# CarbonMatrixLab/AbX

Measured on AMD Instinct MI355X. Metric: diffusion-steps/sec (100 samples, ~350-res complex), higher is better.
Workload: dtype f32; 1 GPU; L352: L=352 (Lab 228 + antigen 124), 100 samples of one complex over 1 GPU(s), 1 step = ScoreNetwork (3 passes) + get_prev + reverse, seeded random weights, ESM off; L=352, samples_total=100, chunk=auto, parallelism=sample-shard x1, no collective in the step

## Files before the change

abx_amd/_lib.py:

```python
import ctypes as C
import os

_HERE = os.path.dirname(os.path.abspath(__file__))
LIB_PATH = os.environ.get('ABX_HIP_LIB') or os.path.join(_HERE, 'csrc', 'libabx_hip.so')

c_f = C.c_void_p
LL = C.c_longlong
I = C.c_int
F = C.c_float


class AbxGemm(C.Structure):
    _fields_ = [
        ('A', c_f), ('sAb', LL), ('sAm', LL), ('sAk', LL),
        ('B', c_f), ('sBb', LL), ('sBk', LL), ('sBn', LL),
        ('C', c_f), ('sCb', LL), ('sCm', LL),
        ('M', I), ('N', I), ('K', I), ('batch', I),
        ('c_transposed', I),
        ('ln_stats', c_f), ('sSb', LL),
        ('ln_csum', c_f),
        ('ln_eps', F),
        ('a_relu', I),
        ('bias', c_f),
        ('alpha', F),
# ... 300 lines not shown
        ('out', c_f), ('out_stride', LL),
        ('bonds', c_f), ('rows', c_f),
        ('B', I), ('L', I), ('Lab', I),
    ]


_S = c_f

_PROTOS = {
    'abx_version': (I, []),
    'abx_last_error_string': (C.c_char_p, []),
    'abx_init': (I, [I]),
    'abx_gemm': (I, [C.POINTER(AbxGemm), _S]),
    'abx_gemm_side': (I, [C.POINTER(AbxGemm), C.POINTER(AbxGemm), _S]),
    'abx_gemm_check_modes': (I, [C.POINTER(AbxGemm)]),
    'abx_gemm_planes_ok': (I, [LL]),
    'abx_split_weights_f16': (I, [c_f, LL, LL, I, I, I, C.c_void_p, _S]),
    'abx_ipa_tail': (I, [C.POINTER(AbxIpaTail), _S]),
    'abx_heads_tail': (I, [C.POINTER(AbxHeadsTail), _S]),
    'abx_gemm3_occupancy': (I, [I]),
    'abx_row_stats': (I, [c_f, LL, LL, LL, I, I, I, F, c_f, _S]),
    'abx_layernorm': (I, [c_f, LL, LL, I, c_f, c_f, F, c_f, LL, c_f, LL, _S]),
    'abx_tri_attn_fwd': (I, [C.POINTER(AbxTriAttn), _S]),
    'abx_tri_rowpack_bytes': (LL, []),
    'abx_tri_rowpack': (I, [C.POINTER(AbxLinearPack), c_f, C.POINTER(AbxTriRowPack), _S]),
    'abx_tri_attn_rowfused_ok': (I, [I]),
    'abx_tri_attn_rowfused_fwd': (I, [C.POINTER(AbxTriAttn), c_f, LL, LL, LL, C.POINTER(AbxTriRowPack), I, _S]),
    'abx_seq_attn_fwd': (I, [c_f, c_f, c_f, c_f, c_f, I, I, I, I, F, _S]),
    'abx_ipa_pack': (I, [c_f, c_f, c_f, c_f, c_f, c_f, I, I, F, _S]),
    'abx_ipa_attn': (I, [c_f, c_f, c_f, c_f, c_f, c_f, c_f, c_f, c_f, c_f, c_f, I, I, _S]),
    'abx_debug_poison_lds': (I, [C.c_uint, _S]),
    'abx_ipa_weights': (I, [c_f, c_f, c_f, c_f, c_f, c_f, c_f, c_f, c_f, c_f, I, I, _S]),
    'abx_ipa_pair': (I, [c_f, c_f, c_f, I, I, _S]),
    'abx_ipa_attn_workspace_bytes': (C.c_longlong, [I, I]),
    'abx_ipa_qpack_bytes': (C.c_longlong, [I, I]),
    'abx_timestep_embedding': (I, [c_f, c_f, I, I, c_f, _S]),
    'abx_assemble_seq': (I, [c_f, LL, c_f, c_f, I, c_f, c_f, c_f, c_f, c_f, I, I, I, I, _S]),
    'abx_assemble_pair': (I, [c_f, LL, c_f, c_f, c_f, c_f, c_f, c_f, c_f, c_f, I, I, I, I, _S]),
    'abx_opm_features': (I, [c_f, c_f, LL, c_f, I, I, I, _S]),
    'abx_opm_out_fwd': (I, [c_f, LL, c_f, c_f, c_f, I, I, c_f, I, _S]),
    'abx_assemble_pair_bias': (I, [c_f, LL, c_f, c_f, c_f, c_f, c_f, c_f, c_f, C.c_void_p, I, c_f, c_f, F, c_f, I, I, c_f, I, _S]),
    'abx_pair_mask': (I, [c_f, c_f, I, I, I, _S]),
    'abx_transpose_last2': (I, [c_f, c_f, I, I, I, I, _S]),
    'abx_pair_embed_features': (I, [c_f, c_f, c_f, c_f, c_f, c_f, c_f, c_f, c_f, c_f, c_f, c_f, I, I, _S]),
    'abx_relpos_block': (I, [c_f, c_f, c_f, I, I, I, I, I, _S]),
    'abx_gather_rows': (I, [c_f, c_f, c_f, c_f, LL, LL, I, _S]),
    'abx_frames_init': (I, [c_f, I, c_f, c_f, c_f, c_f, c_f, c_f, I, F, _S]),
    'abx_rigid_update': (I, [c_f, c_f, c_f, c_f, c_f, c_f, c_f, c_f, I, F, _S]),
    'abx_scores': (I, [C.POINTER(AbxScoreArgs), _S]),
    'abx_torsion_finalize': (I, [c_f, c_f, c_f, c_f, I, _S]),
    'abx_seq_head_atoms': (I, [c_f, c_f, c_f, c_f, c_f, c_f, c_f, c_f, c_f, c_f, c_f, c_f, I, _S]),
    'abx_prev_pos': (I, [c_f, c_f, I, c_f, I, I, _S]),
    'abx_plddt': (I, [c_f, c_f, I, I, _S]),
    'abx_igso3_tables': (I, [c_f, c_f, I, I, I, c_f, c_f, c_f, _S]),
    'abx_reverse_step': (I, [C.POINTER(AbxReverseArgs), _S]),
    'abx_clash_grad_workspace_bytes': (LL, [I, I]),
    'abx_clash_grad': (I, [C.POINTER(AbxGuidanceArgs), c_f, _S]),
    'abx_contact_grad_workspace_bytes': (LL, [I, I, I]),
    'abx_contact_grad': (I, [C.POINTER(AbxContactArgs), c_f, _S]),
    'abx_design_scores_workspace_bytes': (LL, [I, I]),
    'abx_design_scores': (I, [C.POINTER(AbxDesignScoreArgs), c_f, _S]),
    'abx_relax_workspace_bytes': (LL, [I, I, I]),
    'abx_relax_lds_bytes': (LL, [I, I]),
    'abx_relax': (I, [C.POINTER(AbxRelaxArgs), c_f, _S]),
    'abx_interface_scores_workspace_bytes': (LL, [I, I, I]),
    'abx_interface_scores': (I, [C.POINTER(AbxInterfaceArgs), c_f, _S]),
# ... 55 lines not shown
```

abx_amd/csrc/ipa.hip:

```cpp
#include "common.h"
#include "abx_hip.h"

namespace {

constexpr int H = 12, SQK = 16, SV = 16, PQK = 4, PV = 8, CZ = 128;
constexpr int QREC = SQK + 3 * PQK;
constexpr int VREC = SV + 3 * PV;
constexpr int NPROJ = H * SQK + H * (SQK + SV) + 3 * H * PQK + 3 * H * (PQK + PV);
constexpr int OFF_KV = H * SQK;
constexpr int OFF_QP = OFF_KV + H * (SQK + SV);
constexpr int OFF_KVP = OFF_QP + 3 * H * PQK;
constexpr int NFEAT = H * SV + 3 * H * PV + H * PV + H * CZ;

constexpr int IPA_THREADS = 512;
constexpr int IQ = 12;
constexpr int HG = 4, NHG = H / HG;

__global__ __launch_bounds__(256) void ipa_pack_kernel(const float* __restrict__ proj, const float* __restrict__ rots,
                                                       const float* __restrict__ trans, float* __restrict__ qpack,
                                                       float* __restrict__ kpack, float* __restrict__ vpack, int B, int L,
                                                       float w_s) {
    const int NIB = (L + IQ - 1) / IQ, LQ = NIB * IQ;
    const long long idx = (long long)blockIdx.x * 256 + threadIdx.x;
    if (idx >= (long long)B * LQ * H) return;
// ... 26 lines not shown
        float x[3];
#pragma unroll
        for (int r = 0; r < 3; ++r) x[r] = p[OFF_QP + r * (H * PQK) + h * PQK + pt];
#pragma unroll
        for (int r = 0; r < 3; ++r) q[2 * (SQK + pt * 3 + r)] = t[r] + (R[r * 3 + 0] * x[0] + R[r * 3 + 1] * x[1] + R[r * 3 + 2] * x[2]);
    }
#pragma unroll
    for (int pt = 0; pt < PQK + PV; ++pt) {
        float x[3], y[3];
#pragma unroll
        for (int r = 0; r < 3; ++r) x[r] = p[OFF_KVP + r * (H * (PQK + PV)) + h * (PQK + PV) + pt];
#pragma unroll
        for (int r = 0; r < 3; ++r) y[r] = t[r] + (R[r * 3 + 0] * x[0] + R[r * 3 + 1] * x[1] + R[r * 3 + 2] * x[2]);
        if (pt < PQK) {
#pragma unroll
            for (int r = 0; r < 3; ++r) k[SQK + pt * 3 + r] = y[r];
        } else {
#pragma unroll
            for (int r = 0; r < 3; ++r) v[SV + (pt - PQK) * 3 + r] = y[r];
        }
    }
}

__host__ __device__ inline int ipa_row_stride(int L) { return ((L + 31) / 32) * 32 + 12; }
constexpr int RED_I = IQ * 4 + 4;
constexpr int RED_G = (HG * VREC / 4) * RED_I + 4;
__host__ __device__ inline size_t ipa_logits_floats(int L) {
    const size_t lgf = (size_t)IQ * HG * ipa_row_stride(L), redf = (size_t)6 * RED_G;
    return lgf > redf ? lgf : redf;
}

#ifdef IPA_STAMP
__device__ unsigned long long ipa_stamp_buf[1024 * 8];
#define ISTAMP(k) { if (threadIdx.x == 0 && blockIdx.x >= 4096 && blockIdx.x < 5120) ipa_stamp_buf[(blockIdx.x - 4096) * 8 + (k)] = __builtin_amdgcn_s_memtime(); }
#else
#define ISTAMP(k) {}
#endif
__global__ __launch_bounds__(IPA_THREADS, 4) void ipa_weights_kernel(const float* __restrict__ qpack, const float* __restrict__ kpack,
                                                                     const float* __restrict__ vpack, const float* __restrict__ bias2d,
                                                                     const float* __restrict__ mask, const float* __restrict__ rots,
                                                                     const float* __restrict__ trans, const float* __restrict__ pw,
                                                                     float* __restrict__ attn, float* __restrict__ feat, int B, int L) {
    extern __shared__ __attribute__((aligned(16))) float smem[];
    const int LR = ipa_row_stride(L);
    float* lg = smem;
    float* opt = smem + ipa_logits_floats(L);
    const int tid = threadIdx.x, lane = tid & 63, wave = tid >> 6;
    const int NIB = (L + IQ - 1) / IQ, per_b = NIB * NHG;
    const int xcd = blockIdx.x & 7, slot = blockIdx.x >> 3;
    const int full_slots = (B / 8) * per_b;
    int b, wb;
    if (slot < full_slots) {
        b = (slot / per_b) * 8 + xcd;
        wb = slot % per_b;
    } else {
        const int t = (slot - full_slots) * 8 + xcd;
        if (t >= (B % 8) * per_b) return;
        b = (B / 8) * 8 + t / per_b;
        wb = t % per_b;
    }
    const int hg = wb % NHG, h0 = hg * HG;
    const int iblk = wb / NHG;
    const int i0 = iblk * IQ;
    const int niq = min(IQ, L - i0);

    ISTAMP(0)
    {
        typedef float f32x2 __attribute__((ext_vector_type(2)));
        const float* __restrict__ qb = qpack + (((long long)b * NIB + iblk) * H + h0) * (IQ / 2) * (QREC * 2);
        const int wpk = (L + 63) >> 6;
        for (int task = wave; task < HG * wpk; task += IPA_THREADS / 64) {
            const int hl = __builtin_amdgcn_readfirstlane(task / wpk);
            const int j = (task - hl * wpk) * 64 + lane;
            const float* kr = kpack + (((long long)b * H + h0 + hl) * L + min(j, L - 1)) * QREC;
            f32x4 kq[QREC / 4];
#pragma unroll
            for (int c4 = 0; c4 < QREC / 4; ++c4) kq[c4] = *reinterpret_cast<const f32x4*>(kr + c4 * 4);
            const float pwh = pw[h0 + hl];
            const f32x2* __restrict__ qh = reinterpret_cast<const f32x2*>(qb + (long long)hl * (IQ / 2) * (QREC * 2));
#pragma unroll
            for (int ip = 0; ip < IQ / 2; ++ip) {
                f32x2 sacc = {0.f, 0.f}, d2 = {0.f, 0.f};
// ... 144 lines not shown
        }
        if (jg == 0) {
#pragma unroll
            for (int iq = 0; iq < IQ; ++iq) *reinterpret_cast<f32x4*>(opt + (size_t)(iq * HG + hl1) * VREC + c41 * 4) = acc[iq];
        }
        __syncthreads();
    }
    ISTAMP(6)
    for (int idx = tid; idx < niq * HG * SV; idx += IPA_THREADS) {
        const int iq = idx / (HG * SV), r = idx % (HG * SV);
        feat[((long long)b * L + i0 + iq) * NFEAT + h0 * SV + r] = opt[(iq * HG + r / SV) * VREC + (r % SV)];
    }
    for (int idx = tid; idx < niq * HG * PV; idx += IPA_THREADS) {
        const int iq = idx / (HG * PV), nl = idx % (HG * PV);
        const int hl = nl / PV, pt = nl % PV, n = h0 * PV + nl;
        const long long row = (long long)b * L + i0 + iq;
        const float* R = rots + row * 9;
        const float* t = trans + row * 3;
        const float* g = opt + (iq * HG + hl) * VREC + SV + pt * 3;
        float loc[3];
#pragma unroll
        for (int r = 0; r < 3; ++r) {
            const float it = -(R[0 * 3 + r] * t[0] + R[1 * 3 + r] * t[1] + R[2 * 3 + r] * t[2]);
            loc[r] = it + (R[0 * 3 + r] * g[0] + R[1 * 3 + r] * g[1] + R[2 * 3 + r] * g[2]);
        }
        float* fo = feat + row * NFEAT;
#pragma unroll
        for (int r = 0; r < 3; ++r) fo[H * SV + r * (H * PV) + n] = loc[r];
        fo[H * SV + 3 * H * PV + n] = sqrtf(loc[0] * loc[0] + loc[1] * loc[1] + loc[2] * loc[2] + 1e-8f);
    }
    ISTAMP(7)
}

constexpr int PAIR_WAVES = 4;
#ifndef ABX_PAIR_UZ
#define ABX_PAIR_UZ 8
#endif
constexpr int UZ = ABX_PAIR_UZ;

__global__ __launch_bounds__(PAIR_WAVES * 64) void ipa_pair_kernel(const float* __restrict__ attn, const float* __restrict__ z,
                                                                   float* __restrict__ feat, long long rows, int L) {
    typedef float f32x2 __attribute__((ext_vector_type(2)));
    __shared__ __attribute__((aligned(16))) float wl[PAIR_WAVES][UZ * H];
    const int lane = threadIdx.x & 63, wave = threadIdx.x >> 6;
    const long long row = (long long)blockIdx.x * PAIR_WAVES + wave;
    if (row >= rows) return;
    const float* __restrict__ wr = attn + row * L * H;
    const float* __restrict__ zr = z + row * L * CZ + lane * 2;
    float* ws = wl[wave];
    const int nw = L * HG;
    f32x2 acc[H];
#pragma unroll
    for (int h = 0; h < H; ++h) acc[h] = (f32x2){0.f, 0.f};
    f32x2 za[UZ], zb[UZ];
    float wa[NHG], wb[NHG];
    auto request = [&](int j0, f32x2 (&zd)[UZ], float (&wd)[NHG]) {
#pragma unroll
        for (int u = 0; u < UZ; ++u) zd[u] = *reinterpret_cast<const f32x2*>(zr + (long long)min(j0 + u, L - 1) * CZ);
#pragma unroll
        for (int q = 0; q < NHG; ++q) wd[q] = wr[(long long)q * nw + min(j0 * HG + (lane & (UZ * HG - 1)), nw - 1)];
    };
    auto sum_step = [&](int j0, const f32x2 (&zd)[UZ], const float (&wd)[NHG]) {
#pragma unroll
        for (int q = 0; q < NHG; ++q) ws[q * (UZ * HG) + (lane & (UZ * HG - 1))] = wd[q];
        __builtin_amdgcn_fence(__ATOMIC_RELEASE, "wavefront");
        __builtin_amdgcn_wave_barrier();
        __builtin_amdgcn_fence(__ATOMIC_ACQUIRE, "wavefront");
#pragma unroll
        for (int u = 0; u < UZ; ++u) {
            if (j0 + u < L) {
                f32x4 w4[H / 4];
#pragma unroll
                for (int q = 0; q < NHG; ++q) w4[q] = *reinterpret_cast<const f32x4*>(ws + q * (UZ * HG) + u * HG);
#pragma unroll
                for (int h = 0; h < H; ++h) {
                    const float wh = w4[h >> 2][h & 3];
                    acc[h][0] = fmaf(wh, zd[u][0], acc[h][0]);
                    acc[h][1] = fmaf(wh, zd[u][1], acc[h][1]);
                }
            }
        }
        __builtin_amdgcn_fence(__ATOMIC_RELEASE, "wavefront");
        __builtin_amdgcn_wave_barrier();
    };
    request(0, za, wa);
    for (int j0 = 0; j0 < L; j0 += 2 * UZ) {
        if (j0 + UZ < L) request(j0 + UZ, zb, wb);
        sum_step(j0, za, wa);
        if (j0 + UZ < L) {
            if (j0 + 2 * UZ < L) request(j0 + 2 * UZ, za, wa);
            sum_step(j0 + UZ, zb, wb);
        }
    }
    float* fo = feat + row * NFEAT + (H * SV + 4 * H * PV) + lane * 2;
#pragma unroll
    for (int h = 0; h < H; ++h) *reinterpret_cast<f32x2*>(fo + h * CZ) = acc[h];
}

}

extern "C" int abx_ipa_pack(const float* proj, const float* rots, const float* trans, float* qpack, float* kpack,
                            float* vpack, int B, int L, float scalar_weight, hipStream_t st) {
    ABX_REQUIRE(proj && rots && trans && qpack && kpack && vpack && B > 0 && L > 0, "abx_ipa_pack: bad args");
    const long long n = (long long)B * ((L + IQ - 1) / IQ) * IQ * H;
    hipLaunchKernelGGL(ipa_pack_kernel, dim3((unsigned)((n + 255) / 256)), dim3(256), 0, st, proj, rots, trans, qpack, kpack,
                       vpack, B, L, scalar_weight);
    return abx_check_launch("abx_ipa_pack");
}

extern "C" long long abx_ipa_qpack_bytes(int B, int L) {
    return (long long)B * ((L + IQ - 1) / IQ) * IQ * H * QREC * sizeof(float);
}

extern "C" long long abx_ipa_attn_workspace_bytes(int B, int L) {
    return (long long)B * L * L * H * sizeof(float);
}

extern "C" int abx_ipa_weights(const float* qpack, const float* kpack, const float* vpack, const float* bias2d, const float* mask,
                               const float* rots, const float* trans, const float* point_weights, float* attn_ws, float* feat, int B,
                               int L, hipStream_t st) {
    ABX_REQUIRE(qpack && kpack && vpack && bias2d && mask && rots && trans && point_weights && attn_ws && feat, "abx_ipa_weights: null");
    ABX_REQUIRE(B > 0 && L > 0 && B <= 65535 && (long long)B * L < (1ll << 31), "abx_ipa_weights: bad sizes");
    const size_t lds = (ipa_logits_floats(L) + IQ * HG * VREC) * sizeof(float);
    ABX_REQUIRE(lds <= 160 * 1024, "abx_ipa_weights: L too large for LDS-resident logits");
    if (int rc = abx_ensure_dynamic_lds(reinterpret_cast<const void*>(ipa_weights_kernel), 160 * 1024, "abx_ipa_weights")) return rc;
    const long long per_b = (long long)((L + IQ - 1) / IQ) * NHG;
    const long long nwg = 8 * ((B / 8) * per_b + ((B % 8) * per_b + 7) / 8);
    ABX_REQUIRE(nwg < (1LL << 31), "abx_ipa_weights: grid too large");
    hipLaunchKernelGGL(ipa_weights_kernel, dim3((unsigned)nwg), dim3(IPA_THREADS), lds, st, qpack, kpack, vpack, bias2d, mask,
                       rots, trans, point_weights, attn_ws, feat, B, L);
    return abx_check_launch("abx_ipa_weights");
}

#ifdef IPA_STAMP
extern "C" int abx_ipa_stamps(unsigned long long* out) {
    return (int)hipMemcpyFromSymbol(out, HIP_SYMBOL(ipa_stamp_buf), sizeof(unsigned long long) * 1024 * 8);
}
#endif

extern "C" int abx_ipa_pair(const float* attn_ws, const float* z, float* feat, int B, int L, hipStream_t st) {
    ABX_REQUIRE(attn_ws && z && feat && B > 0 && L > 0 && (long long)B * L < (1ll << 31), "abx_ipa_pair: bad args");
    const long long rows = (long long)B * L;
    hipLaunchKernelGGL(ipa_pair_kernel, dim3((unsigned)((rows + PAIR_WAVES - 1) / PAIR_WAVES)), dim3(PAIR_WAVES * 64), 0, st, attn_ws, z,
                       feat, rows, L);
    return abx_check_launch("abx_ipa_pair");
}

extern "C" int abx_ipa_attn(const float* qpack, const float* kpack, const float* vpack, const float* bias2d, const float* z,
                            const float* mask, const float* rots, const float* trans, const float* point_weights, float* attn_ws,
                            float* feat, int B, int L, hipStream_t st) {
    ABX_REQUIRE(z != nullptr, "abx_ipa_attn: null");
    const int rc = abx_ipa_weights(qpack, kpack, vpack, bias2d, mask, rots, trans, point_weights, attn_ws, feat, B, L, st);
    if (rc) return rc;
    return abx_ipa_pair(attn_ws, z, feat, B, L, st);
}
```

abx_amd/model/forward.py:

```python
import math

import numpy as np
import torch

from abx_amd import ops
from abx_amd import residue_constants as rc

_NO_ASSEMBLE_BIAS = not bool(__import__('os').environ.get('ABX_ASSEMBLE_BIAS'))
_NO_OPM_FUSED = bool(__import__('os').environ.get('ABX_NO_OPM_FUSED'))
P_SEQF = 'impl.seqformer.'
P_BLK = 'impl.seqformer.seqformer.blocks.0.'
P_IPA = 'impl.diffusion_module.ScoreNetwork.'


class Packed:

    def __init__(self, sd, device):
        f = lambda k: sd[k].detach().to(device=device, dtype=torch.float32).contiguous()
        self.sd = {k: f(k) for k in sd}
        g = self.sd
        self.wt, self.b = {}, {}
        self._ln_cache = {}
        self._split_cache = {}
        self.gemm_mode = 0
# ... 186 lines not shown
    kw.setdefault('range_class', P.plain_class)
    if narrow and w3 is None and kw['exact'] == 2:
        w3 = P.split_narrow(wt, (name, ln_name))
    return ops.gemm(x, wt, out, bias=bias, ln=(stats, csum), B3=w3, **kw)


class Engine:
    def __init__(self, cfg_model, packed, device):
        self.cfg = cfg_model
        self.P = packed
        self.dev = device
        self.ws = Workspace(device)
        self.block_api = not bool(__import__('os').environ.get('ABX_NO_BLOCK_API'))
        self._blk_ws = {}
        self.fused_heads = not bool(__import__('os').environ.get('ABX_NO_FUSED_HEADS'))
        self.ipa_splitk = int(__import__('os').environ.get('ABX_IPA_SPLITK', '11'))
        c = cfg_model.embeddings_and_seqformer
        pp = c.prev_pos
        self.sq_breaks = torch.square(torch.linspace(pp.min_bin, pp.max_bin, steps=pp.num_bins - 1)).to(device)

    def _block_workspace(self, group, Bc, L):
        key = (group, L)
        hit = self._blk_ws.get(key)
        if hit is None or hit[1] < Bc:
            self._blk_ws = {k: v for k, v in self._blk_ws.items() if k[0] != group}
            buf = ops.tri_attn_block_workspace(Bc, L, self.dev) if group == 'attn' else ops.tri_mul_workspace(Bc, L, self.dev)
            hit = [buf, Bc, Bc]
            self._blk_ws[key] = hit
        elif group == 'mul' and hit[2] != Bc:
            if ((L + 3) // 4 * 4) % 16 != 0:
                ops.tri_mul_workspace_init(hit[0], Bc, L)
            hit[2] = Bc
        return hit[0]

    def static_embeddings(self, batch, shared):
        P, ws = self.P, self.ws
        sl = slice(0, 1) if shared else slice(None)
        seq_t = batch['seq_t'][sl].long().contiguous()
        seq = batch['seq'][sl].long().contiguous()
        B, L = seq.shape
        P.gemm_mode = ops.gemm_mode(L)
        P.plain_class = 'gemm'
        Lab = batch['anchor_flag'].shape[1]
        mask = torch.logical_and(batch['mask'][sl], batch['fixed_mask'][sl].bool())
        mask_f = mask.float().contiguous()
        chain = batch['chain_id'][sl].to(torch.int32).contiguous()
        residx = batch['residx'][sl].to(torch.int32).contiguous()
        atom14 = batch['atom14_gt_positions'][sl].float().contiguous()
        exists = batch['atom14_gt_exists'][sl].to(torch.uint8).contiguous()
        M1, M2 = B * L, B * L * L
        dev = self.dev
        pre = P_SEQF + 'encode_residue_emb.'
        h = torch.empty(M1, 1538, device=dev)
        ops.gather_rows(P.sd[pre + 'aatype_embed.weight'], seq_t, h[:, 0:512], rowscale=mask_f.reshape(-1))
        h[:, 512] = chain.reshape(-1).float()
        h[:, 513] = residx.reshape(-1).float()
        ops.gather_rows(P.sd[pre + 'cdr_embed.weight'], batch['cdr_def'][sl].long().contiguous(), h[:, 514:1026])
        cx = torch.cat([atom14.reshape(M1, 42), batch['torsion_angles_sin_cos'][sl].float().reshape(M1, 14)], dim=-1).contiguous()
        c1 = torch.empty(M1, 512, device=dev)
        _lin(P, pre + 'coordinate_embed.0', cx, c1, act=1)
        _lin(P, pre + 'coordinate_embed.2', c1, h[:, 1026:1538])
        a1 = torch.empty(M1, 1024, device=dev)
        _lin(P, pre + 'mlp.0', h, a1, act=1)
        a2 = torch.empty(M1, 512, device=dev)
        _lin(P, pre + 'mlp.2', a1, a2, act=1)
        a3 = torch.empty(M1, 512, device=dev)
# ... 213 lines not shown
            _ln_lin(P, pre + '1', pre + '0', None, z2, z2, act=1, resid=z2, mlp=P.mlp_second(pre + '3'), exact=2)
        else:
            _ln_lin(P, pre + '1', pre + '0', None, z2, w768, act=1, exact=1)
            _lin(P, pre + '3', w768, z2, resid=z2, exact=1)

        P.plain_class = 'gemm_late'
        ic = cfg.heads.diffusion_module.IPA
        NC = ic.num_channel
        s_pre = ws.get('i_a', (M1, NC))
        _lin(P, P_IPA + 'proj_init_seq_act', s2, s_pre)
        s0 = ws.get('i_s0', (M1, NC))
        ops.layernorm(s_pre, *P.ln(P_IPA + 'init_seq_layer_norm'), out=s0)
        s = ws.get('i_s', (M1, NC))
        _lin(P, P_IPA + 'proj_seq', s0, s)
        zi = w384[:M2 * 128].view(M2, 128)
        if not P.exact('ipa_pair_init'):
            _lin(P, P_IPA + 'proj_init_pair_act', z2, zi, out_ln=P.ln(P_IPA + 'init_pair_layer_norm'), exact=2)
        else:
            _lin(P, P_IPA + 'proj_init_pair_act', z2, zi, exact=1)
            ops.layernorm(zi, *P.ln(P_IPA + 'init_pair_layer_norm'), out=zi)
        bias2d = w384[M2 * 128:M2 * 140].view(M2, 12)
        _lin(P, P_IPA + 'attention_module.proj_pair', zi, bias2d, alpha=P.ipa_w2d, narrow=True)
        attn_ws = w384[M2 * 140:M2 * 152].view(M2, 12)
        init_q = ws.get('f_iq', (M1, 4)); init_t = ws.get('f_it', (M1, 3))
        cur_q = ws.get('f_q', (M1, 4)); cur_t = ws.get('f_t', (M1, 3)); cur_R = ws.get('f_R', (M1, 9))
        delta_q = ws.get('f_dq', (M1, 4))
        rig_in = st['rigids_t'][b0:b1].contiguous()
        ops.frames_init(rig_in, init_q, init_t, cur_q, cur_t, cur_R, delta_q, M1, ic.position_scale)
        proj = ws.get('i_proj', (M1, 1152))
        qpack = ws.get('i_qp', (ops.ipa_qpack_numel(Bc, L),)); kpack = ws.get('i_kp', (M1 * 12 * 28,)); vpack = ws.get('i_vp', (M1 * 12 * 40,))
        ifeat = ws.get('i_feat', (M1, 2112))
        h1 = ws.get('i_h1', (M1, NC)); h2 = ws.get('i_h2', (M1, NC))
        upd = ws.get('i_upd', (M1, 6))
        tail = None
        if not P.exact('ipa_tail', 'gemm_late') and NC == 256:
            wb = lambda n: (P.split(P_IPA + n), P.b[P_IPA + n])
            tail = (wb('attention_module.final_proj'), P.ln(P_IPA + 'attention_layer_norm'), wb('transition_module.0'),
                    wb('transition_module.2'), wb('transition_module.4'), P.ln(P_IPA + 'transition_layer_norm'))
        for _ in range(ic.num_layer):
            _lin(P, P_IPA + 'attention_module.proj', s, proj)
            ops.ipa_pack(proj, cur_R, cur_t, qpack, kpack, vpack, Bc, L, P.ipa_ws)
            ops.ipa_weights(qpack, kpack, vpack, bias2d, mask_f, cur_R, cur_t, P.ipa_pw, attn_ws, ifeat, Bc, L)
            ops.ipa_pair(attn_ws, zi, ifeat, Bc, L)
            if tail is not None:
                part = None
                if self.ipa_splitk and ifeat.shape[1] % (16 * self.ipa_splitk) == 0:
                    part = ops.gemm_splitk(ifeat, tail[0][0], ws.get('i_part', (self.ipa_splitk, M1, NC)), range_class='gemm_late')
                ops.ipa_tail(ifeat, s, *tail, affine=(P.wt[P_IPA + 'affine_update'], P.b[P_IPA + 'affine_update']),
                             rigid=(fixed.reshape(-1), init_q, init_t, cur_q, cur_t, cur_R, delta_q, ic.position_scale), partial=part)
                continue
            else:
                _lin(P, P_IPA + 'attention_module.final_proj', ifeat, s, resid=s)
                ops.layernorm(s, *P.ln(P_IPA + 'attention_layer_norm'), out=s)
                _lin(P, P_IPA + 'transition_module.0', s, h1, act=1)
                _lin(P, P_IPA + 'transition_module.2', h1, h2, act=1)
                _lin(P, P_IPA + 'transition_module.4', h2, s, resid=s)
                ops.layernorm(s, *P.ln(P_IPA + 'transition_layer_norm'), out=s)
            _lin(P, P_IPA + 'affine_update', s, upd)
            ops.rigid_update(upd, fixed.reshape(-1), init_q, init_t, cur_q, cur_t, cur_R, delta_q, M1, ic.position_scale)
        pre = P_IPA + 'sidechain_module.torsion_module.'
        ta = ws.get('t_a', (M1, 128)); tb = ws.get('t_b', (M1, 128))
        un = ws.get('t_un', (M1, 14))
        logits = st['logits'][b0:b1]
        pl = ws.get('h_pl', (M1, 50))
        heads = P.heads_pack() if (self.fused_heads and not P.exact('heads_tail', 'gemm_late') and NC == 256 and ic.torsion.num_residual_block == 2 and
                                   logits.is_contiguous()) else None
        if heads is not None:
            ops.heads_tail(s, s0, heads[0], heads[1], heads[2], un, logits.view(M1, 20), pl if final else None)
        else:
            _lin(P, pre + 'proj_act.1', s, ta, a_relu=True)
            _lin(P, pre + 'proj_init_act.1', s0, ta, a_relu=True, resid=ta)
            for blk in range(ic.torsion.num_residual_block):
                _lin(P, pre + f'blocks.{blk}.net.1', ta, tb, a_relu=True)
                _lin(P, pre + f'blocks.{blk}.net.3', tb, ta, a_relu=True, resid=ta)
            _lin(P, pre + 'projection', ta, un, a_relu=True)
        angles = st['angles'][b0:b1]
        ops.torsion_finalize(un, st['torsion_gt'][b0:b1].contiguous(), fixed.reshape(-1), angles, M1)
        sm = st['structure_module'][b0:b1]
        sm.view(M1, NC).copy_(s)
        t64 = st['t64'][b0:b1].contiguous()
        D = st['diffuser']
        ops.scores(init_q=init_q, init_t=init_t, delta_q=delta_q, cur_t=cur_t, fixed_mask=fixed.reshape(-1), t=t64,
                   t_is_f32=int(st['t_is_f32']), score_norms=D.score_norms, num_sigma=D.num_sigma, num_omega=D.num_omega,
                   discrete_sigma=D.discrete_sigma_dev, discrete_omega=D.discrete_omega_dev,
                   exp_max_sigma=D.exp_max_sigma, exp_min_sigma=D.exp_min_sigma, min_b=D.min_b_f32, bdiff=D.bdiff_f32,
                   coord_scale=D.coord_scale_f32, position_scale=float(ic.position_scale),
                   rot_score=st['rot_score'][b0:b1], trans_score=st['trans_score'][b0:b1], rigids=st['rigids'][b0:b1],
                   B=Bc, L=L)
        pre = 'impl.sequence_module.net.'
        hx = ws.get('h_x', (M1, NC))
        if heads is None:
            ops.layernorm(s, *P.ln(pre + '0'), out=hx)
# ... 16 lines not shown
```

abx_amd/ops.py:

```python
import ctypes as C
import math

import torch

from abx_amd import _lib
from abx_amd._lib import (AbxGemm, AbxTriAttn, AbxIpaTail, AbxHeadsTail, AbxScoreArgs, AbxReverseArgs, AbxGuidanceArgs, AbxContactArgs, AbxDesignScoreArgs, AbxRelaxArgs, AbxInterfaceArgs, AbxPolarArgs, AbxDistogramArgs, AbxAccuracyArgs, AbxEnsemblePairsArgs, AbxEnsembleClusterArgs, AbxLinearPack, AbxLinearSrc,
                           AbxTriMulPack, AbxTriAttnPack, AbxTriRowPack, check)


def _stream():
    return C.c_void_p(torch.cuda.current_stream().cuda_stream)


def _p(t):
    if t is None:
        return None
    assert t.is_cuda, 'libabx_hip works on device memory only'
    return t.data_ptr()


def _f32(t):
    assert t.dtype == torch.float32, t.dtype
    return t

# ... 561 lines not shown
    if RANGE_CHECK and not a.exact:
        a.range_flag, a.range_tag = range_ptr(out.device), RANGE_TAGS['tri_attn']
    if clock_probe is not None:
        assert clock_probe.dtype == torch.int64 and clock_probe.numel() >= 2
        a.clock_probe = _p(clock_probe)
    global _TRI_ATTN_LAST
    _TRI_ATTN_LAST = (int(L), bool(a.exact), fused)
    if fused:
        assert not kv_planes and not a.exact and not tune, 'the row-fused kernel: split-f16, no operand images, no tune bits'
        check(lib.abx_tri_attn_rowfused_fwd(C.byref(a), base, a.sb, a.ss, a.sl, C.byref(rowpack.c), int(slot_order), _stream()), 'abx_tri_attn_rowfused_fwd')
        return out
    check(lib.abx_tri_attn_fwd(C.byref(a), _stream()), 'abx_tri_attn_fwd')
    return out


def seq_attn(qkv, biasT, keymask, gate, out, B, L, H=32, D=17):
    lib = _lib.load()
    assert qkv.is_contiguous() and biasT.is_contiguous() and gate.is_contiguous() and out.is_contiguous()
    check(lib.abx_seq_attn_fwd(_p(qkv), _p(biasT), _p(keymask), _p(gate), _p(out), B, L, H, D, float(D ** (-0.5)), _stream()),
          'abx_seq_attn_fwd')
    return out


def ipa_weights(qpack, kpack, vpack, bias2d, mask, rots, trans, pw, attn_ws, feat, B, L):
    assert attn_ws.numel() >= B * L * L * 12 and attn_ws.is_contiguous()
    check(_lib.load().abx_ipa_weights(_p(qpack), _p(kpack), _p(vpack), _p(bias2d), _p(mask), _p(rots), _p(trans), _p(pw), _p(attn_ws),
                                      _p(feat), B, L, _stream()), 'abx_ipa_weights')


def ipa_pair(attn_ws, z, feat, B, L):
    check(_lib.load().abx_ipa_pair(_p(attn_ws), _p(z), _p(feat), B, L, _stream()), 'abx_ipa_pair')


def gemm_splitk(A, w3, partial, range_class='gemm'):
    S, M, N = partial.shape
    K = A.shape[1]
    assert A.shape[0] == M and A.stride(1) == 1 and partial.is_contiguous() and K % (16 * S) == 0
    _weight_planes(w3, N, K, what='gemm_splitk')
    assert w3.shape[0] * 16 == K
    Ks = K // S
    g = AbxGemm()
    g.A, g.sAb, g.sAm, g.sAk = _p(_f32(A)), Ks, A.stride(0), 1
    g.B_split, g.sB3b, g.sB3k, g.sB3p, g.sB3n = _p(w3), (Ks // 16) * w3.stride(0), w3.stride(0), w3.stride(1), w3.stride(2)
    g.b_f16, g.b_exp = 1, w3.w_exp
    g.C, g.sCb, g.sCm = _p(_f32(partial)), M * N, N
    g.M, g.N, g.K, g.batch = M, N, Ks, S
    g.alpha, g.exact = 1.0, 2
    if RANGE_CHECK:
        g.range_flag, g.range_tag = range_ptr(A.device), RANGE_TAGS[range_class]
    check(_lib.load().abx_gemm(C.byref(g), _stream()), 'abx_gemm(split-K)')
    return partial


def ipa_tail(feat, s, w_final, ln1, w_t0, w_t2, w_t4, ln2, eps=1e-5, affine=None, rigid=None, partial=None):
    M, K1 = feat.shape
    assert s.shape == (M, 256) and feat.stride(1) == 1 and s.stride(1) == 1 and K1 % 16 == 0
    a = AbxIpaTail()
    a.feat, a.s_feat, a.s, a.s_s, a.M, a.K1, a.C = _p(_f32(feat)), feat.stride(0), _p(_f32(s)), s.stride(0), M, K1, 256
    if partial is not None:
        assert partial.dim() == 3 and partial.shape[1:] == (M, 256) and partial.is_contiguous()
        a.partial, a.n_partial, a.s_partial = _p(_f32(partial)), partial.shape[0], M * 256
    for tag, (w3, bias), K in (('final', w_final, K1), ('t0', w_t0, 256), ('t2', w_t2, 256), ('t4', w_t4, 256)):
        _weight_planes(w3, 256, K, what='ipa_tail ' + tag)
        assert w3.shape[0] * 16 == K and bias.numel() == 256
        setattr(a, 'W_' + tag, _p(w3)); setattr(a, 'e_' + tag, w3.w_exp); setattr(a, 'b_' + tag, _p(_f32(bias)))
    a.ln1_w, a.ln1_b, a.ln2_w, a.ln2_b = _p(_f32(ln1[0])), _p(_f32(ln1[1])), _p(_f32(ln2[0])), _p(_f32(ln2[1]))
# ... 604 lines not shown
```

include/abx_hip.h:

```cpp
#ifndef ABX_HIP_H
#define ABX_HIP_H

#include <stdint.h>
#ifdef __HIPCC__
#include <hip/hip_runtime.h>
#else
typedef struct ihipStream_t* hipStream_t;
#endif

#ifdef __cplusplus
extern "C" {
#endif

#define ABX_HIP_ABI_VERSION 1

int abx_version(void);
const char* abx_last_error_string(void);
int abx_init(int device);
int abx_debug_poison_lds(unsigned pattern, hipStream_t stream);

typedef struct AbxGemm {
    const float* A; long long sAb, sAm, sAk;
    const float* B; long long sBb, sBk, sBn;
    float* C;       long long sCb, sCm;
// ... 104 lines not shown
    int tune;
    int bias_log2;
    int kv_planes;
    int q_parts, row_groups;
} AbxTriAttn;
#define ABX_TRI_BIAS_LOG2 (1.4426950408889634f * 128.0f)
int abx_tri_attn_fwd(const AbxTriAttn* desc, hipStream_t stream);

typedef struct AbxTriRowPack {
    const unsigned short* planes;
    const float* csum;
    const float* bias;
    int b_exp;
    int H;
} AbxTriRowPack;
#define ABX_TRI_ROWFUSED_LMAX 352
long long abx_tri_rowpack_bytes(void);
int abx_tri_attn_rowfused_ok(int L);
int abx_tri_attn_rowfused_fwd(const AbxTriAttn* desc, const float* z, long long zb, long long zs, long long zl, const AbxTriRowPack* pack,
                              int slot_order, hipStream_t stream);

int abx_seq_attn_fwd(const float* qkv, const float* bias, const float* keymask, const float* gate, float* out, int B, int L,
                     int H, int D, float scale, hipStream_t stream);

int abx_ipa_pack(const float* proj, const float* rots, const float* trans, float* qpack, float* kpack, float* vpack,
                 int B, int L, float scalar_weight, hipStream_t stream);
int abx_ipa_attn(const float* qpack, const float* kpack, const float* vpack, const float* bias2d, const float* z,
                 const float* mask, const float* rots, const float* trans, const float* point_weights ,
                 float* attn_ws, float* feat, int B, int L, hipStream_t stream);
int abx_ipa_weights(const float* qpack, const float* kpack, const float* vpack, const float* bias2d, const float* mask,
                    const float* rots, const float* trans, const float* point_weights, float* attn_ws, float* feat, int B, int L,
                    hipStream_t stream);
int abx_ipa_pair(const float* attn_ws, const float* z, float* feat, int B, int L, hipStream_t stream);
long long abx_ipa_attn_workspace_bytes(int B, int L);
long long abx_ipa_qpack_bytes(int B, int L);

int abx_timestep_embedding(const double* t, const float* freqs, int B, int dim, float* out, hipStream_t stream);
int abx_assemble_seq(const float* seq_static, long long ss_b, const float* aa_table, const long long* seq_t, int Lab,
                     const float* temb, const float* prev_seq, const float* gamma, const float* beta, float* out, int B,
                     int L, int C, int E, hipStream_t stream);
int abx_assemble_pair(const float* pair_static, long long ps_b, const float* temb, const float* prev_pair,
                      const float* gamma, const float* beta, const long long* prev_pos, const float* pos_table, float* out,
                      float* stats_out, int B, int L, int C, int E, hipStream_t stream);
int abx_assemble_pair_bias(const float* pair_static, long long ps_b, const float* temb, const float* prev_pair, const float* gamma,
                           const float* beta, const long long* prev_pos, const float* pos_table, float* out, const unsigned short* w_planes,
                           int w_exp, const float* csum, const float* bias, float ln_eps, float* biasT, int B, int L, int* range_flag,
                           int range_tag, hipStream_t stream);
int abx_opm_features(const float* left, const float* right, long long ld, float* feat, int B, int L, int C,
                     hipStream_t stream);
int abx_opm_out_fwd(const float* lr, long long ld, const float* Wt, const float* bias, float* z, int B, int L, int* range_flag, int range_tag,
                    hipStream_t stream);
int abx_transpose_last2(const float* in, float* out, int nmat, int L, int Lp, int transpose, hipStream_t stream);
int abx_pair_mask(const float* mask, float* out, int B, int L, int Lp, hipStream_t stream);

int abx_pair_embed_features(const long long* aa, const int* chain_id, const int* residx, const float* atom14,
                            const unsigned char* atom14_exists, const float* aa_pair_embed, const float* relpos_embed,
                            const float* distcoef, const float* dgram_embed, const float* sq_breaks ,
                            float* feat512, float* dist196, int B, int L, hipStream_t stream);
int abx_relpos_block(const int* residx, const float* table, float* out, int B, int L, int Lab, int C, int max_rel,
                     hipStream_t stream);
int abx_gather_rows(const float* table, const long long* idx, const float* rowscale, float* out, long long s_out, long long n,
                    int C, hipStream_t stream);

int abx_frames_init(const void* rigids_t, int is_f64, float* init_q, float* init_t, float* cur_q, float* cur_t, float* cur_R,
                    float* delta_q, int n, float position_scale, hipStream_t stream);
int abx_rigid_update(const float* upd6, const int* fixed_mask, const float* init_q, const float* init_t, float* cur_q,
// ... 259 lines not shown
```

Baseline: 173.8 sample-steps/s.

## Pipeline IPA weights and pair kernels across two batch halves in one launch

```diff
diff --git a/abx_amd/_lib.py b/abx_amd/_lib.py
--- a/abx_amd/_lib.py
+++ b/abx_amd/_lib.py
@@ -356,6 +356,8 @@
     'abx_debug_poison_lds': (I, [C.c_uint, _S]),
     'abx_ipa_weights': (I, [c_f, c_f, c_f, c_f, c_f, c_f, c_f, c_f, c_f, c_f, I, I, _S]),
     'abx_ipa_pair': (I, [c_f, c_f, c_f, I, I, _S]),
+    'abx_ipa_attn_pipelined': (I, [c_f] * 10 + [I, c_f, c_f, c_f, I, I, I, I, _S]),
+    'abx_ipa_pipelined_enabled': (I, []),
     'abx_ipa_attn_workspace_bytes': (C.c_longlong, [I, I]),
     'abx_ipa_qpack_bytes': (C.c_longlong, [I, I]),
     'abx_timestep_embedding': (I, [c_f, c_f, I, I, c_f, _S]),
diff --git a/abx_amd/csrc/ipa.hip b/abx_amd/csrc/ipa.hip
--- a/abx_amd/csrc/ipa.hip
+++ b/abx_amd/csrc/ipa.hip
@@ -82,22 +82,22 @@
 
 #ifdef IPA_STAMP
 __device__ unsigned long long ipa_stamp_buf[1024 * 8];
-#define ISTAMP(k) { if (threadIdx.x == 0 && blockIdx.x >= 4096 && blockIdx.x < 5120) ipa_stamp_buf[(blockIdx.x - 4096) * 8 + (k)] = __builtin_amdgcn_s_memtime(); }
+#define ISTAMP(k) { if (threadIdx.x == 0 && wg >= 4096 && wg < 5120) ipa_stamp_buf[(wg - 4096) * 8 + (k)] = __builtin_amdgcn_s_memtime(); }
 #else
 #define ISTAMP(k) {}
 #endif
-__global__ __launch_bounds__(IPA_THREADS, 4) void ipa_weights_kernel(const float* __restrict__ qpack, const float* __restrict__ kpack,
-                                                                     const float* __restrict__ vpack, const float* __restrict__ bias2d,
-                                                                     const float* __restrict__ mask, const float* __restrict__ rots,
-                                                                     const float* __restrict__ trans, const float* __restrict__ pw,
-                                                                     float* __restrict__ attn, float* __restrict__ feat, int B, int L) {
-    extern __shared__ __attribute__((aligned(16))) float smem[];
+__device__ __forceinline__ void ipa_weights_body(const float* __restrict__ qpack, const float* __restrict__ kpack,
+                                                 const float* __restrict__ vpack, const float* __restrict__ bias2d,
+                                                 const float* __restrict__ mask, const float* __restrict__ rots,
+                                                 const float* __restrict__ trans, const float* __restrict__ pw,
+                                                 float* __restrict__ attn, float* __restrict__ feat, int B, int L, const int wg,
+                                                 float* smem) {
     const int LR = ipa_row_stride(L);
     float* lg = smem;
     float* opt = smem + ipa_logits_floats(L);
     const int tid = threadIdx.x, lane = tid & 63, wave = tid >> 6;
     const int NIB = (L + IQ - 1) / IQ, per_b = NIB * NHG;
-    const int xcd = blockIdx.x & 7, slot = blockIdx.x >> 3;
+    const int xcd = wg & 7, slot = wg >> 3;
     const int full_slots = (B / 8) * per_b;
     int b, wb;
     if (slot < full_slots) {
@@ -308,22 +308,32 @@
     ISTAMP(7)
 }
 
+__global__ __launch_bounds__(IPA_THREADS, 4) void ipa_weights_kernel(const float* __restrict__ qpack, const float* __restrict__ kpack,
+                                                                     const float* __restrict__ vpack, const float* __restrict__ bias2d,
+                                                                     const float* __restrict__ mask, const float* __restrict__ rots,
+                                                                     const float* __restrict__ trans, const float* __restrict__ pw,
+                                                                     float* __restrict__ attn, float* __restrict__ feat, int B, int L) {
+    extern __shared__ __attribute__((aligned(16))) float smem[];
+    ipa_weights_body(qpack, kpack, vpack, bias2d, mask, rots, trans, pw, attn, feat, B, L, (int)blockIdx.x, smem);
+}
+
 constexpr int PAIR_WAVES = 4;
 #ifndef ABX_PAIR_UZ
 #define ABX_PAIR_UZ 8
 #endif
 constexpr int UZ = ABX_PAIR_UZ;
-
-__global__ __launch_bounds__(PAIR_WAVES * 64) void ipa_pair_kernel(const float* __restrict__ attn, const float* __restrict__ z,
-                                                                   float* __restrict__ feat, long long rows, int L) {
+#ifndef ABX_PIPE_UZ
+#define ABX_PIPE_UZ 8
+#endif
+constexpr int PIPE_UZ = ABX_PIPE_UZ;
+
+template <int UZ>
+__device__ __forceinline__ void ipa_pair_body(const float* __restrict__ attn, const float* __restrict__ z, float* __restrict__ feat,
+                                              const long long row, int L, float* ws) {
     typedef float f32x2 __attribute__((ext_vector_type(2)));
-    __shared__ __attribute__((aligned(16))) float wl[PAIR_WAVES][UZ * H];
-    const int lane = threadIdx.x & 63, wave = threadIdx.x >> 6;
-    const long long row = (long long)blockIdx.x * PAIR_WAVES + wave;
-    if (row >= rows) return;
+    const int lane = threadIdx.x & 63;
     const float* __restrict__ wr = attn + row * L * H;
     const float* __restrict__ zr = z + row * L * CZ + lane * 2;
-    float* ws = wl[wave];
     const int nw = L * HG;
     f32x2 acc[H];
 #pragma unroll
@@ -371,6 +381,41 @@
     float* fo = feat + row * NFEAT + (H * SV + 4 * H * PV) + lane * 2;
 #pragma unroll
     for (int h = 0; h < H; ++h) *reinterpret_cast<f32x2*>(fo + h * CZ) = acc[h];
+}
+
+__global__ __launch_bounds__(PAIR_WAVES * 64) void ipa_pair_kernel(const float* __restrict__ attn, const float* __restrict__ z,
+                                                                   float* __restrict__ feat, long long rows, int L) {
+    __shared__ __attribute__((aligned(16))) float wl[PAIR_WAVES][UZ * H];
+    const int wave = threadIdx.x >> 6;
+    const long long row = (long long)blockIdx.x * PAIR_WAVES + wave;
+    if (row >= rows) return;
+    ipa_pair_body<UZ>(attn, z, feat, row, L, wl[wave]);
+}
+
+constexpr int PIPE_PAIR_WAVES = IPA_THREADS / 64;
+__global__ __launch_bounds__(IPA_THREADS, 4) void ipa_pipelined_kernel(
+    const float* __restrict__ qpack, const float* __restrict__ kpack, const float* __restrict__ vpack, const float* __restrict__ bias2d,
+    const float* __restrict__ mask, const float* __restrict__ rots, const float* __restrict__ trans, const float* __restrict__ pw,
+    float* __restrict__ attn_a, float* __restrict__ feat_a, int Ba, const float* __restrict__ attn_b, const float* __restrict__ z_b,
+    float* __restrict__ feat_b, long long rows_b, int L, int n_w, int n_p, int w_run, int p_run, int n_runs) {
+    extern __shared__ __attribute__((aligned(16))) float smem[];
+    const int period = w_run + p_run, g = (int)blockIdx.x;
+    int role_p, idx;
+    if (g < n_runs * period) {
+        const int run = g / period, o = g - run * period;
+        role_p = o >= w_run;
+        idx = role_p ? run * p_run + (o - w_run) : run * w_run + o;
+    } else {
+        role_p = n_runs * w_run >= n_w;
+        idx = (role_p ? n_runs * p_run : n_runs * w_run) + (g - n_runs * period);
+    }
+    if (!role_p) {
+        if (idx < n_w) ipa_weights_body(qpack, kpack, vpack, bias2d, mask, rots, trans, pw, attn_a, feat_a, Ba, L, idx, smem);
+    } else {
+        const int wave = threadIdx.x >> 6;
+        const long long row = (long long)idx * PIPE_PAIR_WAVES + wave;
+        if (idx < n_p && row < rows_b) ipa_pair_body<PIPE_UZ>(attn_b, z_b, feat_b, row, L, smem + wave * (PIPE_UZ * H));
+    }
 }
 
 }
@@ -408,6 +453,43 @@
     return abx_check_launch("abx_ipa_weights");
 }
 
+extern "C" int abx_ipa_pipelined_enabled(void) {
+    static const bool off = [] {
+        const char* e = getenv("ABX_NO_IPA_PIPELINED");
+        return e != nullptr && !(e[0] == '0' && e[1] == 0);
+    }();
+    return off ? 0 : 1;
+}
+
+extern "C" int abx_ipa_attn_pipelined(const float* qpack, const float* kpack, const float* vpack, const float* bias2d, const float* mask,
+                                      const float* rots, const float* trans, const float* point_weights, float* attn_a, float* feat_a,
+                                      int Ba, const float* attn_b, const float* z_b, float* feat_b, int Bb, int L, int w_run, int p_run,
+                                      hipStream_t st) {
+    ABX_REQUIRE(qpack && kpack && vpack && bias2d && mask && rots && trans && point_weights && attn_a && feat_a && attn_b && z_b && feat_b,
+                "abx_ipa_attn_pipelined: null");
+    ABX_REQUIRE(Ba > 0 && Bb > 0 && L > 0 && Ba <= 65535 && (long long)Ba * L < (1ll << 31) && (long long)Bb * L < (1ll << 31),
+                "abx_ipa_attn_pipelined: bad sizes");
+    ABX_REQUIRE(w_run > 0 && p_run > 0 && w_run % 8 == 0 && p_run % 8 == 0 && w_run <= 4096 && p_run <= 4096,
+                "abx_ipa_attn_pipelined: runs must be positive multiples of 8");
+    const size_t lds = (ipa_logits_floats(L) + IQ * HG * VREC) * sizeof(float);
+    ABX_REQUIRE(lds <= 160 * 1024, "abx_ipa_attn_pipelined: L too large for LDS-resident logits");
+    static_assert((size_t)IQ * HG * VREC >= (size_t)PIPE_PAIR_WAVES * PIPE_UZ * H, "slab strips must fit the weights role's LDS");
+    if (int rc = abx_ensure_dynamic_lds(reinterpret_cast<const void*>(ipa_pipelined_kernel), 160 * 1024, "abx_ipa_attn_pipelined")) return rc;
+    const long long per_b = (long long)((L + IQ - 1) / IQ) * NHG;
+    const long long n_w = 8 * ((Ba / 8) * per_b + ((Ba % 8) * per_b + 7) / 8);
+    const long long rows_b = (long long)Bb * L;
+    const long long n_p = (rows_b + PIPE_PAIR_WAVES - 1) / PIPE_PAIR_WAVES;
+    const long long runs_w = (n_w + w_run - 1) / w_run, runs_p = (n_p + p_run - 1) / p_run;
+    const long long n_runs = runs_w < runs_p ? runs_w : runs_p;
+    const long long rest_w = n_w - n_runs * w_run, rest_p = n_p - n_runs * p_run;
+    const long long grid = n_runs * (w_run + p_run) + (rest_w > 0 ? rest_w : rest_p > 0 ? rest_p : 0);
+    ABX_REQUIRE(grid < (1LL << 31), "abx_ipa_attn_pipelined: grid too large");
+    hipLaunchKernelGGL(ipa_pipelined_kernel, dim3((unsigned)grid), dim3(IPA_THREADS), lds, st, qpack, kpack, vpack, bias2d, mask, rots,
+                       trans, point_weights, attn_a, feat_a, Ba, attn_b, z_b, feat_b, rows_b, L, (int)n_w, (int)n_p, w_run, p_run,
+                       (int)n_runs);
+    return abx_check_launch("abx_ipa_attn_pipelined");
+}
+
 #ifdef IPA_STAMP
 extern "C" int abx_ipa_stamps(unsigned long long* out) {
     return (int)hipMemcpyFromSymbol(out, HIP_SYMBOL(ipa_stamp_buf), sizeof(unsigned long long) * 1024 * 8);
diff --git a/abx_amd/model/forward.py b/abx_amd/model/forward.py
--- a/abx_amd/model/forward.py
+++ b/abx_amd/model/forward.py
@@ -242,6 +242,83 @@
                 ops.tri_mul_workspace_init(hit[0], Bc, L)
             hit[2] = Bc
         return hit[0]
+
+    def ipa_tail_pack(self):
+        P = self.P
+        if P.exact('ipa_tail', 'gemm_late'):
+            return None
+        wb = lambda n: (P.split(P_IPA + n), P.b[P_IPA + n])
+        return (wb('attention_module.final_proj'), P.ln(P_IPA + 'attention_layer_norm'), wb('transition_module.0'),
+                wb('transition_module.2'), wb('transition_module.4'), P.ln(P_IPA + 'transition_layer_norm'))
+
+    def ipa_layers(self, num_layer, Bc, L, *, s, zi, bias2d, attn_ws, mask_f, fixed, init_q, init_t, cur_q, cur_t, cur_R, delta_q, proj, qpack,
+                   kpack, vpack, ifeat, h1, h2, upd, tail, position_scale, pipelined=None):
+        P, ws = self.P, self.ws
+        if pipelined is None:
+            pipelined = Bc >= ops.IPA_PIPELINED_MIN_B and ops.ipa_pipelined_enabled()
+
+        def cut(x, lo, n):
+            if lo == 0 and n == Bc:
+                return x
+            per = x.numel() // Bc
+            assert per * Bc == x.numel() and x.is_contiguous()
+            return x.view(-1)[lo * per:(lo + n) * per].view(-1, *x.shape[1:])
+
+        def front(lo, n):
+            _lin(P, P_IPA + 'attention_module.proj', cut(s, lo, n), cut(proj, lo, n))
+            ops.ipa_pack(cut(proj, lo, n), cut(cur_R, lo, n), cut(cur_t, lo, n), cut(qpack, lo, n), cut(kpack, lo, n), cut(vpack, lo, n), n, L,
+                         P.ipa_ws)
+
+        def w_args(lo, n):
+            return (cut(qpack, lo, n), cut(kpack, lo, n), cut(vpack, lo, n), cut(bias2d, lo, n), cut(mask_f, lo, n), cut(cur_R, lo, n),
+                    cut(cur_t, lo, n), P.ipa_pw, cut(attn_ws, lo, n), cut(ifeat, lo, n), n)
+
+        def p_args(lo, n):
+            return (cut(attn_ws, lo, n), cut(zi, lo, n), cut(ifeat, lo, n), n)
+
+        def back(lo, n, tag):
+            f, sh = cut(ifeat, lo, n), cut(s, lo, n)
+            if tail is not None:
+                part = None
+                if self.ipa_splitk and f.shape[1] % (16 * self.ipa_splitk) == 0:
+                    part = ops.gemm_splitk(f, tail[0][0], ws.get('i_part' + tag, (self.ipa_splitk, n * L, sh.shape[1])), range_class='gemm_late')
+                ops.ipa_tail(f, sh, *tail, affine=(P.wt[P_IPA + 'affine_update'], P.b[P_IPA + 'affine_update']),
+                             rigid=(cut(fixed, lo, n), cut(init_q, lo, n), cut(init_t, lo, n), cut(cur_q, lo, n), cut(cur_t, lo, n),
+                                    cut(cur_R, lo, n), cut(delta_q, lo, n), position_scale), partial=part)
+                return
+            a1, a2, u = cut(h1, lo, n), cut(h2, lo, n), cut(upd, lo, n)
+            _lin(P, P_IPA + 'attention_module.final_proj', f, sh, resid=sh)
+            ops.layernorm(sh, *P.ln(P_IPA + 'attention_layer_norm'), out=sh)
+            _lin(P, P_IPA + 'transition_module.0', sh, a1, act=1)
+            _lin(P, P_IPA + 'transition_module.2', a1, a2, act=1)
+            _lin(P, P_IPA + 'transition_module.4', a2, sh, resid=sh)
+            ops.layernorm(sh, *P.ln(P_IPA + 'transition_layer_norm'), out=sh)
+            _lin(P, P_IPA + 'affine_update', sh, u)
+            ops.rigid_update(u, cut(fixed, lo, n), cut(init_q, lo, n), cut(init_t, lo, n), cut(cur_q, lo, n), cut(cur_t, lo, n), cut(cur_R, lo, n),
+                             cut(delta_q, lo, n), n * L, position_scale)
+
+        if not pipelined:
+            for _ in range(num_layer):
+                front(0, Bc)
+                ops.ipa_weights(*w_args(0, Bc), L)
+                ops.ipa_pair(*p_args(0, Bc), L)
+                back(0, Bc, '')
+            return
+        n0 = Bc - Bc // 2
+        H0, H1 = (0, n0), (n0, Bc - n0)
+        for l in range(num_layer):
+            front(*H0)
+            if l == 0:
+                ops.ipa_weights(*w_args(*H0), L)
+            else:
+                ops.ipa_attn_pipelined(*w_args(*H0), *p_args(*H1), L)
+                back(*H1, '1')
+            front(*H1)
+            ops.ipa_attn_pipelined(*w_args(*H1), *p_args(*H0), L)
+            back(*H0, '0')
+        if num_layer > 0:
+            ops.ipa_pair(*p_args(*H1), L)
+            back(*H1, '1')
 
     def static_embeddings(self, batch, shared):
         P, ws = self.P, self.ws
@@ -521,32 +598,10 @@
         ifeat = ws.get('i_feat', (M1, 2112))
         h1 = ws.get('i_h1', (M1, NC)); h2 = ws.get('i_h2', (M1, NC))
         upd = ws.get('i_upd', (M1, 6))
-        tail = None
-        if not P.exact('ipa_tail', 'gemm_late') and NC == 256:
-            wb = lambda n: (P.split(P_IPA + n), P.b[P_IPA + n])
-            tail = (wb('attention_module.final_proj'), P.ln(P_IPA + 'attention_layer_norm'), wb('transition_module.0'),
-                    wb('transition_module.2'), wb('transition_module.4'), P.ln(P_IPA + 'transition_layer_norm'))
-        for _ in range(ic.num_layer):
-            _lin(P, P_IPA + 'attention_module.proj', s, proj)
-            ops.ipa_pack(proj, cur_R, cur_t, qpack, kpack, vpack, Bc, L, P.ipa_ws)
-            ops.ipa_weights(qpack, kpack, vpack, bias2d, mask_f, cur_R, cur_t, P.ipa_pw, attn_ws, ifeat, Bc, L)
-            ops.ipa_pair(attn_ws, zi, ifeat, Bc, L)
-            if tail is not None:
-                part = None
-                if self.ipa_splitk and ifeat.shape[1] % (16 * self.ipa_splitk) == 0:
-                    part = ops.gemm_splitk(ifeat, tail[0][0], ws.get('i_part', (self.ipa_splitk, M1, NC)), range_class='gemm_late')
-                ops.ipa_tail(ifeat, s, *tail, affine=(P.wt[P_IPA + 'affine_update'], P.b[P_IPA + 'affine_update']),
-                             rigid=(fixed.reshape(-1), init_q, init_t, cur_q, cur_t, cur_R, delta_q, ic.position_scale), partial=part)
-                continue
-            else:
-                _lin(P, P_IPA + 'attention_module.final_proj', ifeat, s, resid=s)
-                ops.layernorm(s, *P.ln(P_IPA + 'attention_layer_norm'), out=s)
-                _lin(P, P_IPA + 'transition_module.0', s, h1, act=1)
-                _lin(P, P_IPA + 'transition_module.2', h1, h2, act=1)
-                _lin(P, P_IPA + 'transition_module.4', h2, s, resid=s)
-                ops.layernorm(s, *P.ln(P_IPA + 'transition_layer_norm'), out=s)
-            _lin(P, P_IPA + 'affine_update', s, upd)
-            ops.rigid_update(upd, fixed.reshape(-1), init_q, init_t, cur_q, cur_t, cur_R, delta_q, M1, ic.position_scale)
+        tail = self.ipa_tail_pack() if NC == 256 else None
+        self.ipa_layers(ic.num_layer, Bc, L, s=s, zi=zi, bias2d=bias2d, attn_ws=attn_ws, mask_f=mask_f, fixed=fixed.reshape(-1), init_q=init_q,
+                        init_t=init_t, cur_q=cur_q, cur_t=cur_t, cur_R=cur_R, delta_q=delta_q, proj=proj, qpack=qpack, kpack=kpack, vpack=vpack,
+                        ifeat=ifeat, h1=h1, h2=h2, upd=upd, tail=tail, position_scale=ic.position_scale)
         pre = P_IPA + 'sidechain_module.torsion_module.'
         ta = ws.get('t_a', (M1, 128)); tb = ws.get('t_b', (M1, 128))
         un = ws.get('t_un', (M1, 14))
diff --git a/abx_amd/ops.py b/abx_amd/ops.py
--- a/abx_amd/ops.py
+++ b/abx_amd/ops.py
@@ -617,6 +617,22 @@
     check(_lib.load().abx_ipa_pair(_p(attn_ws), _p(z), _p(feat), B, L, _stream()), 'abx_ipa_pair')
 
 
+IPA_PIPELINED_MIN_B = 16
+IPA_PIPELINED_RUNS = (16, 8)
+
+
+def ipa_pipelined_enabled():
+    return bool(_lib.load().abx_ipa_pipelined_enabled())
+
+
+def ipa_attn_pipelined(qpack, kpack, vpack, bias2d, mask, rots, trans, pw, attn_a, feat_a, Ba, attn_b, z_b, feat_b, Bb, L, runs=None):
+    w_run, p_run = runs or IPA_PIPELINED_RUNS
+    assert attn_a.numel() >= Ba * L * L * 12 and attn_a.is_contiguous() and attn_b.numel() >= Bb * L * L * 12 and attn_b.is_contiguous()
+    check(_lib.load().abx_ipa_attn_pipelined(_p(qpack), _p(kpack), _p(vpack), _p(bias2d), _p(mask), _p(rots), _p(trans), _p(pw), _p(attn_a),
+                                             _p(feat_a), Ba, _p(attn_b), _p(z_b), _p(feat_b), Bb, L, int(w_run), int(p_run), _stream()),
+          'abx_ipa_attn_pipelined')
+
+
 def gemm_splitk(A, w3, partial, range_class='gemm'):
     S, M, N = partial.shape
     K = A.shape[1]
diff --git a/include/abx_hip.h b/include/abx_hip.h
--- a/include/abx_hip.h
+++ b/include/abx_hip.h
@@ -160,6 +160,11 @@
                     const float* rots, const float* trans, const float* point_weights, float* attn_ws, float* feat, int B, int L,
                     hipStream_t stream);
 int abx_ipa_pair(const float* attn_ws, const float* z, float* feat, int B, int L, hipStream_t stream);
+int abx_ipa_attn_pipelined(const float* qpack, const float* kpack, const float* vpack, const float* bias2d, const float* mask,
+                           const float* rots, const float* trans, const float* point_weights, float* attn_a, float* feat_a, int Ba,
+                           const float* attn_b, const float* z_b, float* feat_b, int Bb, int L, int w_run, int p_run,
+                           hipStream_t stream);
+int abx_ipa_pipelined_enabled(void);
 long long abx_ipa_attn_workspace_bytes(int B, int L);
 long long abx_ipa_qpack_bytes(int B, int L);
 
```

Result: no change. 173.4 sample-steps/s (-0.3%).
